# srendle/libfm

Measured on NVIDIA H100. Metric: MovieLens-1M-shaped examples/sec at k=8, SGD, higher is better.
Workload: dtype f32

## Files before the change

libfm_b200/csrc/fm_hogwild.cu:

```cuda
#include <algorithm>

#include "fm_hogwild_common.cuh"
#include "fm_rowgroup.cuh"

namespace fmb {

template <int G, int S, int R, int RW, int U, bool DAMP>
__global__ void __launch_bounds__(HW_MAX_THREADS, row_class_ctas(R, U))
    fm_sgd_hogwild_kernel(const HogwildArgs a) {
  using RG = RowGroup<G, S, R, RW>;
  constexpr int E = RG::E;
  constexpr int RPW = 32 / E;
  extern __shared__ __align__(128) unsigned char smem[];
  uint64_t* bars = reinterpret_cast<uint64_t*>(smem);
  float* s_acc = reinterpret_cast<float*>(smem + 64);

  const int tid = threadIdx.x;
  const int lane = tid & 31;
  const int warp = tid >> 5;
  const int nwarp = blockDim.x >> 5;
  const int rows_per_set = nwarp * RPW;
  const int lig = lane % E;
  const int c = lig % G;
  const int s = lig / G;
  const int sub = lane / E;
  const int TR = a.tile_rows;

  const uint64_t policy = ring_init(smem, tid);
  uint32_t* s_tile = reinterpret_cast<uint32_t*>(smem + 208);
  TileSched sched{a.sched, a.n_tiles, false};
  const int ptid = (int)blockDim.x - 32;
  uint32_t claim_raw = HW_NO_TILE;
  if (tid == ptid) {
    for (int i = 0; i < HW_NSTAGE; i++) {
      const uint32_t t = sched.claim();
      s_tile[i] = t;
      if (t != HW_NO_TILE) {
        const uint64_t r0 = (uint64_t)t * TR, r1 = min(r0 + (uint64_t)TR, a.n_rows);
        issue_tile(a, smem, bars, t, i, policy, __ldg(a.row_ptr + r0), __ldg(a.row_ptr + r1));
      }
    }
    claim_raw = sched.fire();
  }
  __syncthreads();

  const float4* V4 = reinterpret_cast<const float4*>(a.v);
  const bool use_w = a.use_w != 0;
  const bool use_w0 = a.use_w0 != 0;
  const float lr = a.lr;
  const float nlr_regv = -lr * a.regv;
  const float nlr_regw = -lr * a.regw;

  int it = 0;
  for (;; ++it) {
    const int stage = it % HW_NSTAGE;
    const uint32_t parity = (uint32_t)(it / HW_NSTAGE) & 1u;
    const uint64_t tile = s_tile[stage];
    if (tile == HW_NO_TILE) break;
    uint32_t nt = HW_NO_TILE;
    uint64_t nt_nb = 0, nt_ne = 0;
    if (tid == ptid) {
      nt = sched.resolve(claim_raw);
      claim_raw = sched.fire();
      if (nt != HW_NO_TILE) {
        const uint64_t r0 = (uint64_t)nt * TR, r1 = min(r0 + (uint64_t)TR, a.n_rows);
        nt_nb = __ldg(a.row_ptr + r0);
        nt_ne = __ldg(a.row_ptr + r1);
      }
    }
    BiasFetch bias;
    bias.slot = reinterpret_cast<float*>(smem + 192);
    bias.issue(a, use_w0, tid);
    mbar_wait(bars + stage, parity);

    unsigned char* sb = stage_base(smem, a, stage);
    const uint64_t* rp = reinterpret_cast<const uint64_t*>(sb);
    const float* ys = reinterpret_cast<const float*>(sb + (size_t)(TR + 2) * 8);
    const uint32_t* ids = reinterpret_cast<const uint32_t*>(sb + (size_t)(TR + 2) * 8 + (size_t)TR * 4);
    const float* xs = reinterpret_cast<const float*>(ids + a.tile_cap);
    const uint64_t row0 = tile * (uint64_t)TR;
    const int rows_here = (int)min((uint64_t)TR, a.n_rows - row0);
    const uint64_t ab = rp[0] & ~3ull;
    if (a.global_entries) {
      ids = a.col + ab;
      xs = a.val + ab;
    }

    float msum = 0.f, hsum = 0.f;
    float w0 = 0.f;
    bool have_w0 = false;
    for (int rbase = warp * RPW; rbase < rows_here; rbase += U * rows_per_set) {
      RG g[U];
      float y[U];
      bool valid[U];
#pragma unroll
      for (int u = 0; u < U; ++u) {
        const int r = rbase + u * rows_per_set + sub;
        valid[u] = r < rows_here;
        int beg = 0, end = 0;
        y[u] = 0.f;
        if (valid[u]) {
          beg = (int)(rp[r] - ab);
          end = (int)(rp[r + 1] - ab);
          y[u] = ys[r];
        }
        g[u].gather(V4, a.w, a.gp, a.ws, use_w, ids, xs, beg, end, c, s, lig);
      }
      if (!have_w0) {
        w0 = bias.get(use_w0, tid, it, (int)blockDim.x);
        have_w0 = true;
      }
#pragma unroll
      for (int u = 0; u < U; ++u) {
        if (U > 1 && rbase + u * rows_per_set >= rows_here) break;
        RG& gu = g[u];
        const float part = gu.template reduce<DAMP>(V4, a.w, a.gp, a.ws, use_w, ids, xs, c, s, lig);
        const LossStep ls = loss_step(a, w0 + part, y[u]);
        const float mult = ls.mult, curv = ls.curv;
        const float hjoint = DAMP ? curv * ((use_w0 ? 1.f : 0.f) + gu.hrow) : curv;
        if (valid[u] && lig == 0) {
          msum += mult;
          hsum += hjoint;
        }

        const float nlr_mult = -lr * mult;
        auto update_v = [&](int j, const float4& v) {
          const uint32_t id = ids[j];
          const float x = xs[j];
          const float x2 = x * x;
          float sv = 1.f;
          if (DAMP) {
            const float conc = __ldg(a.feat_cnt + id) * a.conc_scale;
            if (conc > 1.f) sv = gamma_scale(conc, lr * (hjoint + a.regv));
          }
          red_add_f4(a.v + ((size_t)id * a.gp + c) * 4,
                     sv * (nlr_mult * (gu.acc.x * x - v.x * x2) + nlr_regv * v.x),
                     sv * (nlr_mult * (gu.acc.y * x - v.y * x2) + nlr_regv * v.y),
                     sv * (nlr_mult * (gu.acc.z * x - v.z * x2) + nlr_regv * v.z),
                     sv * (nlr_mult * (gu.acc.w * x - v.w * x2) + nlr_regv * v.w));
        };
        if (c < a.gp) {
#pragma unroll
          for (int q = 0; q < R; ++q) {
            const int j = gu.beg + s + q * S;
            if (j < gu.end) update_v(j, gu.vc[q]);
          }
          for (int q = R; q < gu.maxit; ++q) {
            const int j = gu.beg + s + q * S;
            if (j < gu.end) update_v(j, ld_cg_f4(V4 + (size_t)ids[j] * a.gp + c));
          }
        }
        auto update_w = [&](int j, float wv) {
          const uint32_t id = ids[j];
          const float x = xs[j];
          float sw = 1.f;
          if (DAMP) {
            const float conc = __ldg(a.feat_cnt + id) * a.conc_scale;
            if (conc > 1.f) sw = gamma_scale(conc, lr * (hjoint + a.regw));
          }
          red_add_f(a.w + (size_t)id * a.ws, sw * (nlr_mult * x + nlr_regw * wv));
        };
        if (use_w) {
#pragma unroll
          for (int t = 0; t < RW; ++t) {
            const int j = gu.beg + lig + t * E;
            if (j < gu.end) update_w(j, gu.wc[t]);
          }
          for (int t = RW; t < gu.maxwit; ++t) {
            const int j = gu.beg + lig + t * E;
            if (j < gu.end) update_w(j, ld_cg_f(a.w + (size_t)ids[j] * a.ws));
          }
        }
      }
    }

    if (!have_w0) w0 = bias.get(use_w0, tid, it, (int)blockDim.x);
    float2* s_part = reinterpret_cast<float2*>(s_acc) + (it & 1) * 8;
    if (use_w0) bias_partial(s_part, msum, hsum, tid);
    __syncthreads();
    if (tid == ptid) {
      s_tile[stage] = nt;
      if (nt != HW_NO_TILE) issue_tile(a, smem, bars, nt, stage, policy, nt_nb, nt_ne);
      if (use_w0) {
        float M = 0.f, H = 0.f;
        for (int i = 0; i < nwarp; i++) {
          M += s_part[i].x;
          H += s_part[i].y;
        }
        const float T = (float)rows_here;
        M += T * a.reg0 * w0;
        const float gsc = gamma_scale(fmaxf(a.w0_conc, 1.f), lr * (H / T + a.reg0));
        red_add_f(a.w0, -lr * gsc * M);
      }
    }
  }
  if (tid == ptid) sched.finish(gridDim.x, claim_raw);
}

using KernelFn = HogwildKernelFn;

template <int G, int S, int CLS>
KernelFn pick_damp(bool damp) {
  constexpr RowClass k = row_class(CLS, G);
  return damp ? fm_sgd_hogwild_kernel<G, S, k.R, k.RW, k.U, true>
              : fm_sgd_hogwild_kernel<G, S, k.R, k.RW, k.U, false>;
}

template <int G, int S>
KernelFn pick_r(int cls, bool damp) {
  switch (cls) {
    case -1: return pick_damp<G, S, -1>(damp);
    case 0: return pick_damp<G, S, 0>(damp);
    case 1: return pick_damp<G, S, 1>(damp);
    case 2: return pick_damp<G, S, 2>(damp);
    default: return pick_damp<G, S, 3>(damp);
  }
}

void pick_geometry(int kp, uint64_t n_rows, uint64_t nnz, int* G, int* S, int* cls) {
  int gp = kp / 4;
  int g = 1;
  while (g < gp) g <<= 1;
  if (g > 32) g = 32;
  double avg = n_rows ? (double)nnz / (double)n_rows : 1.0;
  int s = 1;
  while (s < avg && s < 8) s <<= 1;
  while (g * s > 32) s >>= 1;
  if (s < 1) s = 1;
  *G = g;
  *S = s;
  const int iters = (int)((avg + s - 1) / s);
  *cls = iters <= 1 ? -1 : (iters <= 2 ? 0 : (iters <= 8 ? 1 : ((iters <= 20 || g < 32) ? 2 : 3)));
}

static bool want_damp(const fmb200_ctx* c, const DataSlot& d, double flight_per_sm) {
  const double flight_guess = std::min<double>((double)d.n_rows, (double)c->sm_count * flight_per_sm);
  const double q_max = (double)d.max_feat_cnt * flight_guess / (double)d.n_rows * c->hp.lr *
                       (1.0 + std::max(c->hp.regw, c->hp.regv));
  return c->tune_damp == 1 || (c->tune_damp == 0 && q_max > 0.5);
}

static cudaError_t fit_grid(fmb200_ctx* c, HogwildKernelFn fn, int threads, int smem, uint64_t n_tiles,
                            int* grid) {
  cudaError_t e = cudaFuncSetAttribute(fn, cudaFuncAttributeMaxDynamicSharedMemorySize, smem);
  if (e != cudaSuccess) return e;
  int occ = 0;
  e = cudaOccupancyMaxActiveBlocksPerMultiprocessor(&occ, fn, threads, smem);
  if (e != cudaSuccess) return e;
  if (occ < 1) return cudaErrorInvalidConfiguration;
  const int per_sm = c->tune_ctas_per_sm > 0 ? std::min(c->tune_ctas_per_sm, occ) : occ;
  *grid = (int)std::min<uint64_t>(n_tiles, (uint64_t)c->sm_count * per_sm);
  return cudaSuccess;
}

static HogwildArgs make_args(fmb200_ctx* c, const DataSlot& d, uint64_t n_tiles, int TR,
                             uint32_t tile_cap, uint32_t sbytes) {
  HogwildArgs a;
  a.row_ptr = d.row_ptr.get();
  a.col = d.col.get();
  a.val = d.val.get();
  a.target = d.target.get();
  a.n_rows = d.n_rows;
  a.n_tiles = (uint32_t)n_tiles;
  a.tile_rows = TR;
  a.tile_cap = tile_cap;
  a.stage_bytes = sbytes;
  a.w0 = c->p32.w0();
  a.w = c->p32.w();
  a.v = c->p32.v();
  a.gp = c->kp / 4;
  a.ws = c->p32.ws;
  a.use_w0 = c->k0;
  a.use_w = c->k1;
  a.task = c->hp.task;
  a.lr = (float)c->hp.lr;
  a.reg0 = (float)c->hp.reg0;
  a.regw = (float)c->hp.regw;
  a.regv = (float)c->hp.regv;
  a.min_target = (float)c->hp.min_target;
  a.max_target = (float)c->hp.max_target;
  a.feat_cnt = d.feat_cnt.get();
  a.conc_scale = 1.f;
  a.w0_conc = 1.f;
  a.acc_w0 = a.acc_w = a.acc_v = a.acc_bad = a.acc = nullptr;
  a.state = nullptr;
  a.n_acc = 0;
  a.ramp_tiles = 0;
  a.ramp_conc_scale = a.ramp_w0_conc = 1.f;
  a.gbar = nullptr;
  a.gbar_base = 0;
  a.prof = nullptr;
  a.deal_pos = nullptr;
  a.bias_rows = nullptr;
  a.acc_w0x = nullptr;
  a.sched = c->d_sched.get();
  a.global_entries = 0;
  return a;
}

static unsigned long long* acc_flag(fmb200_ctx* c) { return c->d_acc.get() + c->p32.n_floats; }

cudaError_t clear_acc_flag(fmb200_ctx* c) {
  return c->d_acc ? cudaMemsetAsync(acc_flag(c), 0, sizeof(unsigned long long), c->stream) : cudaSuccess;
}

struct RowlaneShape {
  HogwildKernelFn fn = nullptr;
  uint32_t cap = 0, sbytes = 0;
  int smem = 0;
};
static RowlaneShape rowlane_shape(HogwildKernelFn fn, int TR, uint32_t cap, int hdr_bytes) {
  const uint32_t sbytes = (uint32_t)hw_stage_bytes(TR, cap);
  return RowlaneShape{fn, cap, sbytes, hdr_bytes + HW_NSTAGE * (int)sbytes};
}

struct RowlanePlan {
  int threads = 0, TR = 0, launch_threads = 0, grid = 0;
  bool damp = false, combine = false, ws = false, prof = false, dealable = false;
  RowlaneShape file, dealt;
};

static cudaError_t plan_rowlane(fmb200_ctx* c, const DataSlot& d, RowlanePlan* p, bool* ok) {
  *ok = false;
  const int gp = c->kp / 4;
  if (gp < 1 || gp > 2 || d.max_row_nnz > 4 || c->tune_variant == 1 || d.n_rows == 0) return cudaSuccess;
  int threads = c->tune_threads > 0 ? std::min(c->tune_threads, HW_MAX_THREADS) : 256;
  int tr_idx = 0;
  while ((32 << (tr_idx + 1)) <= threads) tr_idx++;
  p->threads = 32 << tr_idx;
  p->TR = p->threads;
  p->damp = want_damp(c, d, 3.0 * p->TR);
  p->combine = (double)d.max_feat_cnt * 32.0 / (double)d.n_rows > 0.5;
  p->ws = c->tune_variant == 3;
  p->prof = c->tune_variant == 132 || c->tune_variant == 133;
  const uint32_t cap = (d.tile_span[tr_idx] + 3u) & ~3u;
  p->file = rowlane_shape(pick_rowlane_kernel(gp, (int)d.max_row_nnz, p->ws, p->damp, p->combine, p->prof, false),
                          p->TR, cap, p->ws ? HW_WS_HDR_BYTES : HW_HDR_BYTES);
  if (p->file.fn == nullptr) return cudaSuccess;
  p->launch_threads = p->ws ? p->threads + 32 : p->threads;
  const uint64_t n_tiles = (d.n_rows + p->TR - 1) / p->TR;
  cudaError_t e = fit_grid(c, p->file.fn, p->launch_threads, p->file.smem, n_tiles, &p->grid);
  if (e != cudaSuccess) return e;
  *ok = true;
  if (p->ws || p->combine || c->tune_variant == 5 || c->tune_variant == 133) return cudaSuccess;
  p->dealt = rowlane_shape(pick_rowlane_kernel(gp, (int)d.max_row_nnz, false, p->damp, false, p->prof, true), p->TR,
                           std::max<uint32_t>(cap, (uint32_t)p->TR * d.max_row_nnz + 4u), HW_HDR_BYTES);
  int grid_dealt = 0;
  if ((e = fit_grid(c, p->dealt.fn, p->threads, p->dealt.smem, n_tiles, &grid_dealt)) != cudaSuccess) return e;
  p->dealable = grid_dealt == p->grid;
  return cudaSuccess;
}

cudaError_t prepare_rowlane_deal(fmb200_ctx* c, DataSlot& d) {
  if (c->mode != FMB200_MODE_HOGWILD || c->kp == 0) return cudaSuccess;
  RowlanePlan p;
  bool ok = false;
  cudaError_t e = plan_rowlane(c, d, &p, &ok);
  if (e != cudaSuccess || !ok || !p.dealable) return e;
  return build_rowlane_deal(c, d, p.TR, (uint32_t)p.grid);
}

static cudaError_t launch_rowlane(fmb200_ctx* c, DataSlot& d, bool* handled) {
  *handled = false;
  RowlanePlan p;
  bool ok = false;
  cudaError_t e = plan_rowlane(c, d, &p, &ok);
  if (e != cudaSuccess || !ok) return e;
  const int TR = p.TR;
  const int grid = p.grid;
  const uint64_t n_tiles = (d.n_rows + TR - 1) / TR;
  const bool ws = p.ws;
  constexpr uint64_t kRampTiles = 4;
  const bool ramp = c->hogwild_fresh && c->k0 && c->tune_damp >= 0 && n_tiles > 8 * kRampTiles;
  c->hogwild_fresh = false;
  const bool dealt = p.dealable && !ramp && (d.deal.matches(d.upload_gen, TR, (uint32_t)grid) || d.hogwild_epochs > 0);
  d.hogwild_epochs++;
  const RowlaneShape& shape = dealt ? p.dealt : p.file;
  const HogwildKernelFn fn = shape.fn;
  const int smem = shape.smem;
  const int launch_threads = p.launch_threads;
  HogwildArgs a = make_args(c, d, n_tiles, TR, shape.cap, shape.sbytes);
  a.conc_scale = (float)(std::min<double>((double)d.n_rows, (double)grid * TR) / (double)d.n_rows);
  a.w0_conc = (float)std::min<double>((double)d.n_rows, (double)grid * TR * (ws ? HW_NSTAGE : 1));
  if (ws) {
    if (ramp) {
      HogwildArgs r = a;
      r.n_rows = kRampTiles * (uint64_t)TR;
      r.n_tiles = (uint32_t)kRampTiles;
      r.conc_scale = (float)((double)TR / (double)d.n_rows);
      r.w0_conc = (float)TR;
      fn<<<1, launch_threads, smem, c->stream>>>(r);
      c->launches++;
      const uint64_t skip = kRampTiles * (uint64_t)TR;
      a.row_ptr += skip;
      a.target += skip;
      a.n_rows -= skip;
      a.n_tiles = (uint32_t)(n_tiles - kRampTiles);
    }
    fn<<<grid, launch_threads, smem, c->stream>>>(a);
    c->launches++;
  } else {
    const uint64_t n_acc = c->p32.n_floats;
    if (n_acc % 4 != 0) return cudaErrorInvalidValue;
    if (!c->d_acc) {
      if ((e = alloc(c->d_acc, n_acc + 1)) != cudaSuccess) return e;
      e = cudaMemsetAsync(c->d_acc.get(), 0, (n_acc + 1) * sizeof(unsigned long long), c->stream);
      if (e != cudaSuccess) return e;
    }
    unsigned long long* acc = c->d_acc.get();
    float* base = c->p32.base;
    a.acc_w0 = acc + (a.w0 - base);
    a.acc_w = acc + (a.w - base);
    a.acc_v = acc + (a.v - base);
    a.acc_bad = acc_flag(c);
    a.state = base;
    a.acc = acc;
    a.n_acc = n_acc;
    if (ramp) {
      a.ramp_tiles = (uint32_t)kRampTiles;
      a.ramp_conc_scale = (float)((double)TR / (double)d.n_rows);
      a.ramp_w0_conc = (float)TR;
    }
    if (dealt) {
      if ((e = build_rowlane_deal(c, d, TR, (uint32_t)grid)) != cudaSuccess) return e;
      a.row_ptr = d.deal.row_ptr.get();
      a.col = d.deal.col.get();
      a.val = d.deal.val.get();
      a.target = d.deal.target.get();
      a.deal_pos = d.deal.pos.get();
      const uint64_t words = 2 + (uint64_t)grid * TR;
      if (c->deal_bias_cap < words) {
        if ((e = grow(c->d_deal_bias, c->deal_bias_cap, words)) != cudaSuccess) return e;
        if ((e = cudaMemsetAsync(c->d_deal_bias.get(), 0, 2 * sizeof(unsigned long long), c->stream)) != cudaSuccess)
          return e;
      }
      a.acc_w0x = c->d_deal_bias.get();
      a.bias_rows = reinterpret_cast<float2*>(c->d_deal_bias.get() + 2);
    }
    a.gbar = c->d_gbar.get();
    a.gbar_base = c->gbar_count;
    PhaseTimers prof;
    if (p.prof && (e = prof.start(RL_PROF_SLOTS, c->stream)) != cudaSuccess) return e;
    a.prof = prof.slots.get();
    void* args[] = {&a};
    e = cudaLaunchCooperativeKernel((const void*)fn, dim3(grid), dim3(launch_threads), args, (size_t)smem,
                                    c->stream);
    if (e != cudaSuccess) return e;
    c->launches++;
    const uint32_t n_win = rowlane_windows(a.n_tiles, a.ramp_tiles, (uint32_t)grid);
    c->gbar_count += (uint32_t)grid * rowlane_barriers(a.n_tiles, a.ramp_tiles, (uint32_t)grid, dealt);
    if (p.prof) {
      static const char* name[RL_PROF_SLOTS] = {"bias+gather", "score+issue", "bulk_wait", "barrier1", "fold",
                                                "barrier2"};
      if ((e = prof.print(c->stream, name, (double)n_win * grid, 1, false,
                          "[rowlane phases, cycles per window of CTA thread 0 (%u windows x %d CTAs)]", n_win,
                          grid)) != cudaSuccess)
        return e;
    }
  }
  c->last_cfg = EpochConfig{1, (int)std::max<uint32_t>(1, d.max_row_nnz), TR, grid, launch_threads, smem,
                            p.damp ? 1 : 0, dealt ? 1 : 0};
  *handled = true;
  return cudaGetLastError();
}

cudaError_t launch_sgd_hogwild(fmb200_ctx* c, DataSlot& d) {
  if (c->kp / 4 > 32) return cudaErrorInvalidValue;
  if (d.n_rows == 0) return cudaSuccess;
  {
    bool handled = false;
    cudaError_t e = launch_rowlane(c, d, &handled);
    if (e != cudaSuccess || handled) return e;
  }
  int G, S, cls;
  pick_geometry(c->kp, d.n_rows, d.nnz, &G, &S, &cls);
  const RowClass rc = row_class(cls, G);
  const int threads = c->tune_threads > 0 ? std::min(c->tune_threads, HW_MAX_THREADS) : 256;
  const int ctas_target = row_class_ctas(rc.R, rc.U);

  const int budget = (c->max_smem_optin - 1024) / ctas_target;
  int tr_idx = 3;
  if (c->tune_rows_per_tile > 0) {
    tr_idx = 0;
    while (tr_idx < 4 && (32 << (tr_idx + 1)) <= c->tune_rows_per_tile) tr_idx++;
  }
  auto stage_bytes_for = [&](int idx) {
    return hw_stage_bytes(32 << idx, ((uint64_t)d.tile_span[idx] + 3u) & ~3ull);
  };
  while (tr_idx > 0 && (uint64_t)HW_HDR_BYTES + HW_NSTAGE * stage_bytes_for(tr_idx) > (uint64_t)budget) tr_idx--;
  const bool global_entries =
      (uint64_t)HW_HDR_BYTES + (uint64_t)HW_NSTAGE * stage_bytes_for(tr_idx) > (uint64_t)c->max_smem_optin;
  if (global_entries) tr_idx = 1;
  const int TR = 32 << tr_idx;
  const uint32_t cap = global_entries ? 0u : (d.tile_span[tr_idx] + 3u) & ~3u;
  const uint32_t sbytes = (uint32_t)hw_stage_bytes(TR, cap);
  const int smem = HW_HDR_BYTES + HW_NSTAGE * (int)sbytes;

  const double rows_per_cta_step = (double)(threads / 32) * (32.0 / (G * S)) * rc.U;
  const bool damp = want_damp(c, d, ctas_target * rows_per_cta_step);

  const KernelFn fn = dispatch_gs(G, S, [&](auto g, auto s) { return pick_r<g, s>(cls, damp); });
  const uint64_t n_tiles = (d.n_rows + TR - 1) / TR;
  int grid = 0;
  cudaError_t e = fit_grid(c, fn, threads, smem, n_tiles, &grid);
  if (e != cudaSuccess) return e;

  HogwildArgs a = make_args(c, d, n_tiles, TR, cap, sbytes);
  a.global_entries = global_entries ? 1 : 0;
  a.conc_scale = (float)(std::min<double>((double)d.n_rows, (double)grid * rows_per_cta_step) /
                         (double)d.n_rows);
  a.w0_conc = (float)std::min<double>((double)d.n_rows, (double)grid * TR);
  fn<<<grid, threads, smem, c->stream>>>(a);
  c->launches++;
  c->last_cfg = EpochConfig{G, S, TR, grid, threads, smem, damp ? 1 : 0};
  return cudaGetLastError();
}

}
```

libfm_b200/csrc/fm_hogwild_common.cuh:

```cuda
#pragma once
#include "fm_device.cuh"
#include "fmb200_internal.h"

namespace fmb {

constexpr int HW_NSTAGE = 3;
constexpr int HW_MAX_THREADS = 256;
constexpr uint32_t HW_NO_TILE = 0xffffffffu;
constexpr int HW_HDR_BYTES = 256;
constexpr int HW_WS_HDR_BYTES = 512;

template <typename T>
__host__ __device__ inline T hw_rp_bytes(int TR) { return (T)(TR + 2) * 8; }
template <typename T>
__host__ __device__ inline T hw_y_bytes(int TR) { return (T)TR * 4; }
__host__ __device__ inline uint64_t hw_stage_bytes(int TR, uint64_t cap) {
  return (hw_rp_bytes<uint64_t>(TR) + hw_y_bytes<uint64_t>(TR) + 2 * cap * 4 + 15) & ~15ull;
}

struct HogwildArgs {
  const uint64_t* row_ptr;
  const uint32_t* col;
  const float* val;
  const float* target;
  uint64_t n_rows;
  uint32_t n_tiles;
  int tile_rows;
  uint32_t tile_cap;
  uint32_t stage_bytes;
  float* w0;
  float* w;
  float* v;
  int gp;
  int ws;
  int use_w0, use_w, task;
  float lr, reg0, regw, regv, min_target, max_target;
  const float* feat_cnt;
  float conc_scale;
  float w0_conc;
  unsigned int* sched;
  int global_entries;
  unsigned long long *acc_w0, *acc_w, *acc_v;
  unsigned long long* acc_bad;
  float* state;
  unsigned long long* acc;
  uint64_t n_acc;
  uint32_t ramp_tiles;
  float ramp_conc_scale, ramp_w0_conc;
  unsigned int* gbar;
  uint32_t gbar_base;
  unsigned long long* prof;
  const uint32_t* deal_pos;
  float2* bias_rows;
  unsigned long long* acc_w0x;
};

__host__ __device__ inline uint32_t rowlane_windows(uint32_t n_tiles, uint32_t ramp, uint32_t G) {
  return ramp + (n_tiles - ramp + G - 1) / G;
}
__host__ __device__ inline uint32_t rowlane_barriers(uint32_t n_tiles, uint32_t ramp, uint32_t G, bool dealt) {
  return 2u * rowlane_windows(n_tiles, ramp, G) - (dealt ? 0u : 1u);
}

struct GridBarrier {
  unsigned int* count;
  uint32_t target;
  __device__ __forceinline__ void arrive(int tid) {
    __syncthreads();
    if (tid == 0) red_release_add_u32(count, 1u);
    target += gridDim.x;
  }
  __device__ __forceinline__ void wait(int tid) {
    if (tid == 0)
      while ((int32_t)(ld_acquire_u32(count) - target) < 0) {
      }
    __syncthreads();
  }
};

constexpr float kAccScale = 0x1p32f;
constexpr float kAccStepMax = 0x1p11f;

__device__ __forceinline__ void acc_add(unsigned long long* p, float d, unsigned long long* bad) {
  if (fabsf(d) < kAccStepMax) red_add_u64(p, (unsigned long long)__float2ll_rn(d * kAccScale));
  else atomicOr(bad, 1ull);
}
__device__ __forceinline__ unsigned long long acc_quantise(float d, unsigned long long* bad) {
  if (fabsf(d) < kAccStepMax) return (unsigned long long)__float2ll_rn(d * kAccScale);
  atomicOr(bad, 1ull);
  return 0ull;
}

__device__ __forceinline__ float acc_fold(float x, unsigned long long u, bool bad) {
  if (bad) return __int_as_float(0x7fffffff);
  return u != 0ull ? x + (float)((double)(long long)u * (1.0 / (double)kAccScale)) : x;
}

__device__ __forceinline__ unsigned char* stage_base(unsigned char* smem, const HogwildArgs& a,
                                                     int stage, int hdr = HW_HDR_BYTES) {
  return smem + hdr + (size_t)stage * a.stage_bytes;
}

__device__ __forceinline__ void issue_tile(const HogwildArgs& a, unsigned char* smem, uint64_t* bars,
                                           uint32_t tile, int stage, uint64_t policy, uint64_t nb,
                                           uint64_t ne, int hdr = HW_HDR_BYTES) {
  const int TR = a.tile_rows;
  const uint64_t r0 = (uint64_t)tile * TR;
  const uint64_t ab = nb & ~3ull;
  const uint64_t ae = (ne + 3ull) & ~3ull;
  const uint32_t ebytes = a.global_entries ? 0u : (uint32_t)(ae - ab) * 4u;
  const uint32_t rp_bytes = hw_rp_bytes<uint32_t>(TR);
  const uint32_t y_bytes = hw_y_bytes<uint32_t>(TR);
  unsigned char* sb = stage_base(smem, a, stage, hdr);
  uint64_t* bar = bars + stage;
  mbar_arrive_expect_tx(bar, rp_bytes + y_bytes + 2u * ebytes);
  bulk_g2s_hint(sb, a.row_ptr + r0, rp_bytes, bar, policy);
  bulk_g2s_hint(sb + rp_bytes, a.target + r0, y_bytes, bar, policy);
  if (ebytes) {
    unsigned char* cb = sb + rp_bytes + y_bytes;
    bulk_g2s_hint(cb, a.col + ab, ebytes, bar, policy);
    bulk_g2s_hint(cb + (size_t)a.tile_cap * 4u, a.val + ab, ebytes, bar, policy);
  }
}

__device__ __forceinline__ uint64_t ring_init(unsigned char* smem, int tid) {
  uint64_t* bars = reinterpret_cast<uint64_t*>(smem);
  uint64_t policy = 0;
  if (tid == 0) {
    for (int i = 0; i < HW_NSTAGE; i++) mbar_init(bars + i, 1);
    fence_mbar_init();
  }
  if (tid == (int)blockDim.x - 32) policy = policy_evict_first();
  __syncthreads();
  return policy;
}

struct LossStep {
  float mult, curv;
};
__device__ __forceinline__ LossStep loss_step(const HogwildArgs& a, float p, float y) {
  LossStep l;
  if (a.task == FMB200_TASK_REGRESSION) {
    const float pc = fmaxf(a.min_target, fminf(a.max_target, p));
    l.mult = pc - y;
    const float den = p - y;
    l.curv = (pc == p) ? 1.f : (fabsf(den) > 1e-12f ? fminf(fmaxf(l.mult / den, 0.f), 1.f) : 0.f);
  } else {
    const float sg = 1.f / (1.f + __expf(-y * p));
    l.mult = -y * (1.f - sg);
    l.curv = sg * (1.f - sg);
  }
  return l;
}

__device__ __forceinline__ float gamma_scale(float c, float u) {
  if (c <= 1.f || u <= 0.f) return 1.f;
  const float q = c * u;
  if (q < 1e-3f) return 1.f;
  const float a = fmaxf(1.f - u, 0.f);
  const float ac = a > 0.f ? __expf(c * __logf(a)) : 0.f;
  return fminf(1.f, (1.f - ac) / q);
}

__device__ __forceinline__ void bias_partial(float2* part, float mult, float hjoint, int tid) {
  mult = warp_sum(mult);
  hjoint = warp_sum(hjoint);
  if ((tid & 31) == 0) part[tid >> 5] = make_float2(mult, hjoint);
}

struct BiasFetch {
  float* slot;
  float pending;
  __device__ __forceinline__ void issue(const HogwildArgs& a, bool use_w0, int tid) {
    pending = 0.f;
    if (use_w0 && tid == 0) pending = ld_cg_f(a.w0);
  }
  __device__ __forceinline__ float get(bool use_w0, int tid, int it, int nthreads) {
    if (!use_w0) return 0.f;
    float* s = slot + (it & 1);
    if (tid < 32) {
      const float v = __shfl_sync(0xffffffffu, pending, 0);
      if (tid == 0) *s = v;
      __threadfence_block();
      named_bar_arrive(1, nthreads);
      return v;
    }
    named_bar_sync(1, nthreads);
    return *s;
  }
};

struct TileSched {
  unsigned int* w;
  uint32_t n_tiles;
  bool dry;
  __device__ __forceinline__ uint32_t claim() {
    if (dry) return HW_NO_TILE;
    const uint32_t t = atomicAdd(w, 1u);
    if (t >= n_tiles) {
      dry = true;
      return HW_NO_TILE;
    }
    return t;
  }
  __device__ __forceinline__ uint32_t fire() { return dry ? HW_NO_TILE : atomicAdd(w, 1u); }
  __device__ __forceinline__ uint32_t resolve(uint32_t raw) {
    if (raw >= n_tiles) {
      dry = true;
      return HW_NO_TILE;
    }
    return raw;
  }
  __device__ __forceinline__ void finish(unsigned int n_ctas, uint32_t last_raw) {
    unsigned int inc = (last_raw == 0x7fffffffu) ? 2u : 1u;
    __threadfence();
    if (atomicAdd(w + 1, inc) == n_ctas - 1) {
      w[0] = 0u;
      w[1] = 0u;
    }
  }
};

using HogwildKernelFn = void (*)(const HogwildArgs);

HogwildKernelFn pick_rowlane_kernel(int gp, int max_row_nnz, bool ws, bool damp, bool combine, bool prof, bool dealt);
constexpr int RL_PROF_SLOTS = 6;

}
```

libfm_b200/csrc/fm_rowlane.cu:

```cuda
#include <algorithm>

#include "fm_hogwild_common.cuh"

namespace fmb {

template <int GP>
struct FactorRow {
  float v[4 * GP];
};

template <int GP>
__device__ __forceinline__ unsigned long long* wb_slot(int e, int tid) {
  __shared__ __align__(128) unsigned long long s_wb[2][HW_MAX_THREADS][4 * GP];
  return s_wb[e & 1][tid];
}
template <int GP, int Z, typename Q>
__device__ __forceinline__ void acc_add_row_q(unsigned long long* acc_v, uint32_t id, bool live, int e, int tid, Q q) {
  constexpr int K = 4 * GP;
  unsigned long long* slot = wb_slot<GP>(e, tid);
  bulk_wait_read<Z == 1 ? 0 : 1>();
  if (live) {
#pragma unroll
    for (int f = 0; f < K; f += 2) *reinterpret_cast<ulonglong2*>(slot + f) = make_ulonglong2(q(f), q(f + 1));
    fence_proxy_async_shared();
    bulk_red_add_u64(acc_v + (size_t)id * K, slot, K * 8);
  }
  bulk_commit();
}
template <int GP, int Z>
__device__ __forceinline__ void acc_add_row(unsigned long long* acc_v, uint32_t id, bool live,
                                            const float (&d)[4 * GP], int e, int tid, unsigned long long* bad) {
  acc_add_row_q<GP, Z>(acc_v, id, live, e, tid, [&](int f) { return acc_quantise(d[f], bad); });
}

template <int GP>
__device__ __forceinline__ FactorRow<GP> gather_row(const float4* V4, uint32_t gid, int odd) {
  FactorRow<GP> r;
  const float4 zero4 = make_float4(0.f, 0.f, 0.f, 0.f);
  if constexpr (GP == 2) {
    const uint32_t pid = __shfl_xor_sync(0xffffffffu, gid, 1);
    const uint32_t idA = odd ? pid : gid;
    const uint32_t idB = odd ? gid : pid;
    const float4 la = idA != 0xffffffffu ? ld_cg_f4(V4 + (size_t)idA * 2 + odd) : zero4;
    const float4 lb = idB != 0xffffffffu ? ld_cg_f4(V4 + (size_t)idB * 2 + odd) : zero4;
    const float4 send = odd ? la : lb;
    float4 recv;
    recv.x = __shfl_xor_sync(0xffffffffu, send.x, 1);
    recv.y = __shfl_xor_sync(0xffffffffu, send.y, 1);
    recv.z = __shfl_xor_sync(0xffffffffu, send.z, 1);
    recv.w = __shfl_xor_sync(0xffffffffu, send.w, 1);
    const float4 lo = odd ? recv : la;
    const float4 hi = odd ? lb : recv;
    r.v[0] = lo.x; r.v[1] = lo.y; r.v[2] = lo.z; r.v[3] = lo.w;
    r.v[4] = hi.x; r.v[5] = hi.y; r.v[6] = hi.z; r.v[7] = hi.w;
  } else {
    const float4 l = gid != 0xffffffffu ? ld_cg_f4(V4 + (size_t)gid) : zero4;
    r.v[0] = l.x; r.v[1] = l.y; r.v[2] = l.z; r.v[3] = l.w;
  }
  return r;
}

template <int GP, int Z, bool DAMP, bool COMBINE, bool ACC, bool DEALT, typename W0F>
__device__ __forceinline__ void rowlane_tile(const HogwildArgs& a, const uint64_t* rp,
                                             const float* ys, const uint32_t* ids,
                                             const float* xs, int rows_here, int tid, W0F get_w0,
                                             float& mult_out, float& hjoint_out) {
  constexpr int K = 4 * GP;
  const int lane = tid & 31;
  const int odd = lane & 1;
  const float4* V4 = reinterpret_cast<const float4*>(a.v);
  const bool use_w = a.use_w != 0;
  const bool use_w0 = a.use_w0 != 0;
  const float lr = a.lr;
  const uint64_t ab = rp[0] & ~3ull;
  const bool valid = tid < rows_here;
  int beg = 0, cnt = 0;
  float y = 0.f;
  if (valid) {
    beg = (int)(rp[tid] - ab);
    cnt = (int)(rp[tid + 1] - ab) - beg;
    y = ys[tid];
  }
  uint32_t id[Z];
  float x[Z], wv[Z];
  FactorRow<GP> vr[Z];
#pragma unroll
  for (int e = 0; e < Z; ++e) {
    const bool on = e < cnt;
    id[e] = on ? ids[beg + e] : 0u;
    x[e] = on ? xs[beg + e] : 0.f;
  }
  const int kq = DEALT ? cnt - 1 : -1;
  uint32_t kid = 0xffffffffu;
#pragma unroll
  for (int e = 0; e < Z; ++e)
    if (e == kq) kid = id[e];
  int seg = lane;
  if (DEALT) {
    const uint32_t prev = __shfl_up_sync(0xffffffffu, kid, 1);
    const bool head = lane == 0 || kid == 0xffffffffu || prev != kid;
    seg = 31 - __clz(__ballot_sync(0xffffffffu, head) & (0xffffffffu >> (31 - lane)));
  }
#pragma unroll
  for (int e = 0; e < Z; ++e) {
    const bool fetch = e < cnt && e != kq;
    vr[e] = gather_row<GP>(V4, fetch ? id[e] : 0xffffffffu, odd);
    wv[e] = (use_w && fetch) ? ld_cg_f(a.w + (size_t)id[e] * a.ws) : 0.f;
  }
  if (DEALT) {
    const bool fetch = lane == seg && kid != 0xffffffffu;
    FactorRow<GP> kv = gather_row<GP>(V4, fetch ? kid : 0xffffffffu, odd);
    float kw = (use_w && fetch) ? ld_cg_f(a.w + (size_t)kid * a.ws) : 0.f;
#pragma unroll
    for (int f = 0; f < K; ++f) kv.v[f] = __shfl_sync(0xffffffffu, kv.v[f], seg);
    kw = __shfl_sync(0xffffffffu, kw, seg);
#pragma unroll
    for (int e = 0; e < Z; ++e)
      if (e == kq) {
        vr[e] = kv;
        wv[e] = kw;
      }
  }

  float sum[K];
#pragma unroll
  for (int f = 0; f < K; ++f) sum[f] = 0.f;
  float sq = 0.f, lin = 0.f, xx = 0.f;
#pragma unroll
  for (int e = 0; e < Z; ++e) {
#pragma unroll
    for (int f = 0; f < K; ++f) {
      const float d = vr[e].v[f] * x[e];
      sum[f] += d;
      sq += d * d;
    }
    lin += wv[e] * x[e];
    xx += x[e] * x[e];
  }
  float s2 = 0.f;
#pragma unroll
  for (int f = 0; f < K; ++f) s2 += sum[f] * sum[f];
  const float w0 = get_w0();
  const float p = w0 + lin + 0.5f * (s2 - sq);

  const LossStep ls = loss_step(a, p, y);
  float mult = ls.mult, curv = ls.curv;
  if (!valid) {
    mult = 0.f;
    curv = 0.f;
  }
  const float hrow = (use_w ? xx : 0.f) + fmaxf((xx - 2.f) * s2 + sq, 0.f);
  const float hjoint = DAMP ? curv * ((use_w0 ? 1.f : 0.f) + hrow) : curv;

  struct KeyStep {
    float v[K], w;
  } kd{};
  auto make_kd = [](const float (&d)[K], float dw) {
    KeyStep k;
#pragma unroll
    for (int f = 0; f < K; ++f) k.v[f] = d[f];
    k.w = dw;
    return k;
  };
  const float nlr_mult = -lr * mult;
  const float nlr_regv = -lr * a.regv;
  const float nlr_regw = -lr * a.regw;
#pragma unroll
  for (int e = 0; e < Z; ++e) {
    const bool on = e < cnt;
    float sv = 1.f, sw = 1.f;
    if (DAMP) {
      const float conc = on ? __ldg(a.feat_cnt + id[e]) * a.conc_scale : 0.f;
      if (conc > 1.f) {
        sv = gamma_scale(conc, lr * (hjoint + a.regv));
        sw = gamma_scale(conc, lr * (hjoint + a.regw));
      }
    }
    const float x2 = x[e] * x[e];
    float d[K];
#pragma unroll
    for (int f = 0; f < K; ++f)
      d[f] = sv * (nlr_mult * (sum[f] * x[e] - vr[e].v[f] * x2) + nlr_regv * vr[e].v[f]);
    float dw = sw * (nlr_mult * x[e] + nlr_regw * wv[e]);
    bool on_c = on;
    if (DEALT && e == kq) {
      kd = make_kd(d, dw);
      on_c = false;
    }
    if (COMBINE) {
      const uint32_t key = on ? id[e] : (0x80000000u | (uint32_t)lane);
      unsigned peers = __match_any_sync(0xffffffffu, key);
      if (__any_sync(0xffffffffu, __popc(peers) > 1)) {
        const int first = __ffs(peers) - 1;
        int rel = __popc(peers << (31 - lane) << 1);
        peers &= (0xfffffffeu << lane);
        while (__any_sync(0xffffffffu, peers != 0u)) {
          const int next = __ffs(peers);
          const int src = next ? next - 1 : lane;
#pragma unroll
          for (int f = 0; f < K; ++f) {
            const float t = __shfl_sync(0xffffffffu, d[f], src);
            if (next) d[f] += t;
          }
          const float tw = __shfl_sync(0xffffffffu, dw, src);
          if (next) dw += tw;
          const unsigned done = __ballot_sync(0xffffffffu, rel & 1);
          peers &= ~done;
          rel >>= 1;
        }
        on_c = on && (lane == first);
      }
    }
    if constexpr (ACC) {
      acc_add_row<GP, Z>(a.acc_v, id[e], on_c, d, e, tid, a.acc_bad);
    } else if (GP == 2) {
      const uint32_t pid = __shfl_xor_sync(0xffffffffu, id[e], 1);
      const bool pon = __shfl_xor_sync(0xffffffffu, (int)on_c, 1) != 0;
      const uint32_t idA = odd ? pid : id[e];
      const uint32_t idB = odd ? id[e] : pid;
      const bool onA = odd ? pon : on_c;
      const bool onB = odd ? on_c : pon;
      float4 send, keep;
      if (odd) {
        send = make_float4(d[0], d[1], d[2], d[3]);
        keep = make_float4(d[4], d[5], d[6], d[7]);
      } else {
        send = make_float4(d[4], d[5], d[6], d[7]);
        keep = make_float4(d[0], d[1], d[2], d[3]);
      }
      float4 recv;
      recv.x = __shfl_xor_sync(0xffffffffu, send.x, 1);
      recv.y = __shfl_xor_sync(0xffffffffu, send.y, 1);
      recv.z = __shfl_xor_sync(0xffffffffu, send.z, 1);
      recv.w = __shfl_xor_sync(0xffffffffu, send.w, 1);
      const float4 va = odd ? recv : keep;
      const float4 vb = odd ? keep : recv;
      if (onA) red_add_f4(a.v + ((size_t)idA * 2 + odd) * 4, va.x, va.y, va.z, va.w);
      if (onB) red_add_f4(a.v + ((size_t)idB * 2 + odd) * 4, vb.x, vb.y, vb.z, vb.w);
    } else if (on_c) {
      red_add_f4(a.v + (size_t)id[e] * 4, d[0], d[1], d[2], d[3]);
    }
    if (on_c && use_w) {
      if (ACC) acc_add(a.acc_w + (size_t)id[e] * a.ws, dw, a.acc_bad);
      else red_add_f(a.w + (size_t)id[e] * a.ws, dw);
    }
  }
  if constexpr (DEALT) {
    const bool has_key = kid != 0xffffffffu;
    unsigned long long q[K + 1];
#pragma unroll
    for (int f = 0; f < K; ++f) q[f] = has_key ? acc_quantise(kd.v[f], a.acc_bad) : 0ull;
    q[K] = (has_key && use_w) ? acc_quantise(kd.w, a.acc_bad) : 0ull;
#pragma unroll
    for (int s = 1; s < 32; s <<= 1) {
      const bool take = __shfl_down_sync(0xffffffffu, seg, s) == seg && lane + s < 32;
#pragma unroll
      for (int f = 0; f <= K; ++f) {
        const unsigned long long t = __shfl_down_sync(0xffffffffu, q[f], s);
        if (take) q[f] += t;
      }
    }
    const bool issue = has_key && lane == seg;
    acc_add_row_q<GP, Z>(a.acc_v, kid, issue, Z, tid, [&](int f) { return q[f]; });
    if (issue && use_w) red_add_u64(a.acc_w + (size_t)kid * a.ws, q[K]);
  }

  mult_out = mult;
  hjoint_out = valid ? hjoint : 0.f;
}

constexpr int RL_PROF_OFF = 200;

template <int GP, int Z, bool DAMP, bool COMBINE, bool PROF, bool DEALT>
__global__ void __launch_bounds__(HW_MAX_THREADS, 3) fm_sgd_rowlane_kernel(const HogwildArgs a) {
  extern __shared__ __align__(128) unsigned char smem[];
  uint64_t* bars = reinterpret_cast<uint64_t*>(smem);
  float* s_acc = reinterpret_cast<float*>(smem + 64);
  unsigned long long* s_prof = reinterpret_cast<unsigned long long*>(smem + RL_PROF_OFF);

  const int tid = threadIdx.x;
  const int TR = a.tile_rows;
  const uint32_t G = gridDim.x;
  const uint32_t R = a.ramp_tiles;
  const uint32_t n_win = rowlane_windows(a.n_tiles, R, G);
  long long tprof = 0;
  auto prof_mark = [&](int slot) {
    if constexpr (PROF) {
      if (tid == 0) {
        const long long now = clock64();
        s_prof[slot] += (unsigned long long)(now - tprof);
        tprof = now;
      }
    }
  };
  if (PROF && tid < RL_PROF_SLOTS) s_prof[tid] = 0ull;
  auto tile_of = [&](uint32_t j) -> uint32_t {
    const uint32_t t = j < R ? (blockIdx.x == 0 ? j : HW_NO_TILE) : R + (j - R) * G + blockIdx.x;
    return t < a.n_tiles ? t : HW_NO_TILE;
  };

  const uint64_t policy = ring_init(smem, tid);
  const int ptid = (int)blockDim.x - 32;
  uint32_t pj = 0;
  auto next_tile = [&]() -> uint32_t {
    for (; pj < n_win; ++pj)
      if (tile_of(pj) != HW_NO_TILE) return tile_of(pj++);
    return HW_NO_TILE;
  };
  if (tid == ptid) {
    for (int i = 0; i < HW_NSTAGE; i++) {
      const uint32_t t = next_tile();
      if (t != HW_NO_TILE) {
        const uint64_t r0 = (uint64_t)t * TR, r1 = min(r0 + (uint64_t)TR, a.n_rows);
        issue_tile(a, smem, bars, t, i, policy, __ldg(a.row_ptr + r0), __ldg(a.row_ptr + r1));
      }
    }
  }
  __syncthreads();

  const bool use_w0 = a.use_w0 != 0;
  const float lr = a.lr;
  GridBarrier gbar{a.gbar, a.gbar_base};
  const uint64_t q0 = blockIdx.x * (uint64_t)blockDim.x + tid;
  const uint64_t fold_stride = (uint64_t)G * blockDim.x;
  const uint64_t n_vec = a.n_acc / 4;
  float4* state4 = reinterpret_cast<float4*>(a.state);
  ulonglong2* acc2 = reinterpret_cast<ulonglong2*>(a.acc);
  if (PROF && tid == 0) tprof = clock64();

  float w0_run = (DEALT && use_w0 && tid == 0) ? ld_cg_f(a.w0) : 0.f;
  bool bad = false;
  int it = 0;
  for (uint32_t j = 0; j < n_win; ++j) {
    const uint32_t tile = tile_of(j);
    if (DEALT && use_w0 && tid == 0 && j > 0) w0_run = acc_fold(w0_run, __ldcg(a.acc_w0x + ((j - 1) & 1)), bad);
    if (tile != HW_NO_TILE) {
      const int stage = it % HW_NSTAGE;
      const uint32_t parity = (uint32_t)(it / HW_NSTAGE) & 1u;
      uint32_t nt = HW_NO_TILE;
      uint64_t nt_nb = 0, nt_ne = 0;
      if (tid == ptid) {
        nt = next_tile();
        if (nt != HW_NO_TILE) {
          const uint64_t r0 = (uint64_t)nt * TR, r1 = min(r0 + (uint64_t)TR, a.n_rows);
          nt_nb = __ldg(a.row_ptr + r0);
          nt_ne = __ldg(a.row_ptr + r1);
        }
      }
      HogwildArgs w = a;
      if (j < R) {
        w.conc_scale = a.ramp_conc_scale;
        w.w0_conc = a.ramp_w0_conc;
      }
      BiasFetch bias;
      bias.slot = reinterpret_cast<float*>(smem + 192);
      if (DEALT) bias.pending = w0_run;
      else bias.issue(a, use_w0, tid);
      const uint32_t pos = DEALT && tid < (int)min((uint64_t)TR, a.n_rows - (uint64_t)tile * TR)
                               ? __ldg(a.deal_pos + (uint64_t)tile * TR + tid)
                               : 0xffffffffu;
      mbar_wait(bars + stage, parity);

      unsigned char* sb = stage_base(smem, a, stage);
      const uint64_t* rp = reinterpret_cast<const uint64_t*>(sb);
      const float* ys = reinterpret_cast<const float*>(sb + (size_t)(TR + 2) * 8);
      const uint32_t* ids = reinterpret_cast<const uint32_t*>(sb + (size_t)(TR + 2) * 8 + (size_t)TR * 4);
      const float* xs = reinterpret_cast<const float*>(ids + a.tile_cap);
      const uint64_t row0 = (uint64_t)tile * TR;
      const int rows_here = (int)min((uint64_t)TR, a.n_rows - row0);

      float mult, hj, w0 = 0.f;
      rowlane_tile<GP, Z, DAMP, COMBINE, true, DEALT>(
          w, rp, ys, ids, xs, rows_here, tid,
          [&]() {
            w0 = bias.get(use_w0, tid, it, (int)blockDim.x);
            prof_mark(0);
            return w0;
          },
          mult, hj);
      float2* s_part = reinterpret_cast<float2*>(s_acc) + (it & 1) * 8;
      if (DEALT) {
        if (use_w0 && pos != 0xffffffffu) a.bias_rows[pos] = make_float2(mult, hj);
      } else if (use_w0) {
        bias_partial(s_part, mult, hj, tid);
      }
      __syncthreads();
      if (tid == ptid) {
        if (nt != HW_NO_TILE) issue_tile(a, smem, bars, nt, stage, policy, nt_nb, nt_ne);
        if (!DEALT && use_w0) {
          float M = 0.f, H = 0.f;
          for (int i = 0; i < (int)(blockDim.x >> 5); i++) {
            M += s_part[i].x;
            H += s_part[i].y;
          }
          const float T = (float)rows_here;
          M += T * a.reg0 * w0;
          const float gsc = gamma_scale(fmaxf(w.w0_conc, 1.f), lr * (H / T + a.reg0));
          acc_add(a.acc_w0, -lr * gsc * M, a.acc_bad);
        }
      }
      ++it;
    }
    prof_mark(1);
    bulk_wait_all();
    fence_proxy_async_global();
    gbar.arrive(tid);
    prof_mark(2);
    float4 s = make_float4(0.f, 0.f, 0.f, 0.f);
    if (q0 < n_vec) s = __ldcg(state4 + q0);
    gbar.wait(tid);
    prof_mark(3);
    float2 pr = make_float2(0.f, 0.f);
    if (DEALT && use_w0 && tile != HW_NO_TILE && tid < (int)min((uint64_t)TR, a.n_rows - (uint64_t)tile * TR))
      pr = __ldcg(a.bias_rows + blockIdx.x * TR + tid);
    bad = __ldcg(a.acc + a.n_acc) != 0ull;
    for (uint64_t q = q0; q < n_vec; q += fold_stride) {
      const ulonglong2 lo = __ldcg(acc2 + 2 * q), hi = __ldcg(acc2 + 2 * q + 1);
      if (q != q0) s = __ldcg(state4 + q);
      s.x = acc_fold(s.x, lo.x, bad);
      s.y = acc_fold(s.y, lo.y, bad);
      s.z = acc_fold(s.z, hi.x, bad);
      s.w = acc_fold(s.w, hi.y, bad);
      if (bad || (lo.x | lo.y | hi.x | hi.y) != 0ull) state4[q] = s;
      if ((lo.x | lo.y) != 0ull) acc2[2 * q] = make_ulonglong2(0ull, 0ull);
      if ((hi.x | hi.y) != 0ull) acc2[2 * q + 1] = make_ulonglong2(0ull, 0ull);
    }
    if (DEALT && use_w0) {
      if (tile != HW_NO_TILE) {
        float2* s_part = reinterpret_cast<float2*>(s_acc);
        bias_partial(s_part, pr.x, pr.y, tid);
        __syncthreads();
        if (tid == 0) {
          float M = 0.f, H = 0.f;
          for (int i = 0; i < (int)(blockDim.x >> 5); i++) {
            M += s_part[i].x;
            H += s_part[i].y;
          }
          const float T = (float)min((uint64_t)TR, a.n_rows - (uint64_t)tile * TR);
          M += T * a.reg0 * w0_run;
          const float gsc = gamma_scale(fmaxf(a.w0_conc, 1.f), lr * (H / T + a.reg0));
          acc_add(a.acc_w0x + (j & 1), -lr * gsc * M, a.acc_bad);
        }
      }
      if (blockIdx.x == 0 && tid == 0 && j > 0) a.acc_w0x[(j - 1) & 1] = 0ull;
    }
    prof_mark(4);
    if (DEALT || j + 1 < n_win) {
      gbar.arrive(tid);
      gbar.wait(tid);
    }
    fence_proxy_async_global();
    prof_mark(5);
  }
  if (DEALT) {
    const bool bad_end = __ldcg(a.acc + a.n_acc) != 0ull;
    if (bad_end && !bad)
      for (uint64_t q = q0; q < n_vec; q += fold_stride) state4[q] = make_float4(NAN, NAN, NAN, NAN);
    if (use_w0 && blockIdx.x == 0 && tid == 0) {
      *a.w0 = acc_fold(w0_run, __ldcg(a.acc_w0x + ((n_win - 1) & 1)), bad_end);
      a.acc_w0x[(n_win - 1) & 1] = 0ull;
    }
  }
  if constexpr (PROF) {
    __syncthreads();
    if (tid < RL_PROF_SLOTS) atomicAdd(a.prof + tid, s_prof[tid]);
  }
}


__device__ __forceinline__ void mbar_arrive(uint64_t* bar) {
  asm volatile("mbarrier.arrive.shared::cta.b64 _, [%0];" ::"r"(smem_u32(bar)) : "memory");
}

template <int GP, int Z, bool DAMP, bool COMBINE>
__global__ void __launch_bounds__(HW_MAX_THREADS + 32, 3) fm_sgd_rowlane_ws_kernel(const HogwildArgs a) {
  extern __shared__ __align__(128) unsigned char smem[];
  uint64_t* full = reinterpret_cast<uint64_t*>(smem);
  uint64_t* empty = reinterpret_cast<uint64_t*>(smem + 64);
  uint32_t* s_tile = reinterpret_cast<uint32_t*>(smem + 128);
  float* s_w0 = reinterpret_cast<float*>(smem + 160);
  float2* s_part = reinterpret_cast<float2*>(smem + 192);

  const int tid = threadIdx.x;
  const int lane = tid & 31;
  const int TR = a.tile_rows;
  const int n_cwarps = TR >> 5;
  const bool use_w0 = a.use_w0 != 0;
  auto stage_ptr = [&](int stage) { return smem + HW_WS_HDR_BYTES + (size_t)stage * a.stage_bytes; };

  if (tid == 0) {
    for (int i = 0; i < HW_NSTAGE; i++) {
      mbar_init(full + i, 1);
      mbar_init(empty + i, (uint32_t)n_cwarps);
    }
    fence_mbar_init();
  }
  __syncthreads();

  if (tid >= TR) {
    if (lane != 0) return;
    TileSched sched{a.sched, a.n_tiles, false};
    const uint64_t policy = policy_evict_first();
    auto fill = [&](int stage, uint32_t t) {
      s_tile[stage] = t;
      if (t == HW_NO_TILE) {
        mbar_arrive(full + stage);
        return;
      }
      s_w0[stage] = use_w0 ? ld_cg_f(a.w0) : 0.f;
      const uint64_t r0 = (uint64_t)t * TR, r1 = min(r0 + (uint64_t)TR, a.n_rows);
      issue_tile(a, smem, full, t, stage, policy, __ldg(a.row_ptr + r0), __ldg(a.row_ptr + r1), HW_WS_HDR_BYTES);
    };
    for (int i = 0; i < HW_NSTAGE; i++) fill(i, sched.claim());
    for (int it = 0;; ++it) {
      const int stage = it % HW_NSTAGE;
      const uint32_t t = s_tile[stage];
      if (t == HW_NO_TILE) break;
      mbar_wait(empty + stage, (uint32_t)(it / HW_NSTAGE) & 1u);
      if (use_w0) {
        float M = 0.f, H = 0.f;
        for (int i = 0; i < n_cwarps; i++) {
          const float2 p = s_part[stage * 8 + i];
          M += p.x;
          H += p.y;
        }
        const uint64_t row0 = (uint64_t)t * TR;
        const float T = (float)min((uint64_t)TR, a.n_rows - row0);
        M += T * a.reg0 * s_w0[stage];
        const float gsc = gamma_scale(fmaxf(a.w0_conc, 1.f), a.lr * (H / T + a.reg0));
        red_add_f(a.w0, -a.lr * gsc * M);
      }
      fill(stage, sched.claim());
    }
    sched.finish(gridDim.x, 0u);
    return;
  }

  for (int it = 0;; ++it) {
    const int stage = it % HW_NSTAGE;
    mbar_wait(full + stage, (uint32_t)(it / HW_NSTAGE) & 1u);
    const uint32_t tile = s_tile[stage];
    if (tile == HW_NO_TILE) break;
    unsigned char* sb = stage_ptr(stage);
    const uint64_t* rp = reinterpret_cast<const uint64_t*>(sb);
    const float* ys = reinterpret_cast<const float*>(sb + (size_t)(TR + 2) * 8);
    const uint32_t* ids = reinterpret_cast<const uint32_t*>(sb + (size_t)(TR + 2) * 8 + (size_t)TR * 4);
    const float* xs = reinterpret_cast<const float*>(ids + a.tile_cap);
    const uint64_t row0 = (uint64_t)tile * TR;
    const int rows_here = (int)min((uint64_t)TR, a.n_rows - row0);
    const float w0 = s_w0[stage];
    float mult, hj;
    rowlane_tile<GP, Z, DAMP, COMBINE, false, false>(a, rp, ys, ids, xs, rows_here, tid, [&]() { return w0; }, mult,
                                                     hj);
    if (use_w0) bias_partial(s_part + stage * 8, mult, hj, tid);
    __syncwarp();
    if (lane == 0) mbar_arrive(empty + stage);
  }
}

template <auto... Vs, class T, class F>
static HogwildKernelFn dispatch(T v, F f) {
  HogwildKernelFn fn = nullptr;
  (void)((v == Vs && (fn = f(std::integral_constant<decltype(Vs), Vs>{}), true)) || ...);
  return fn;
}

HogwildKernelFn pick_rowlane_kernel(int gp, int max_row_nnz, bool ws, bool damp, bool combine, bool prof, bool dealt) {
  const int z = max_row_nnz <= 1 ? 1 : (max_row_nnz <= 2 ? 2 : (max_row_nnz <= 4 ? 4 : 0));
  return dispatch<1, 2>(gp, [&](auto GP) {
    return dispatch<1, 2, 4>(z, [&](auto Z) {
      return dispatch<false, true>(damp, [&](auto D) {
        return dispatch<false, true>(combine, [&](auto C) {
          if (ws) return fm_sgd_rowlane_ws_kernel<GP, Z, D, C>;
          return dispatch<false, true>(prof, [&](auto P) {
            return dispatch<false, true>(dealt, [&](auto DL) -> HogwildKernelFn {
              if constexpr (DL && C) return nullptr;
              else return fm_sgd_rowlane_kernel<GP, Z, D, C, P, DL>;
            });
          });
        });
      });
    });
  });
}

}
```

Before: 6.883 billion.

## Move dealt-mode w0 bias reduction off the grid barrier critical path

In the dealt rowlane path, each CTA's global-bias partial reduction now runs between the grid barrier's arrive and wait, so it overlaps barrier latency. A per-window arrival counter is added, and each CTA spins on it before folding the previous window's w0 accumulator. The fold is deferred into the bias fetch callback instead of happening at window start. This takes the per-window w0 reduction out of the serialized barrier phase, at the cost of an extra counter, spin-waits, and added complexity in resetting the counters.

```diff
diff --git a/libfm_b200/csrc/fm_hogwild.cu b/libfm_b200/csrc/fm_hogwild.cu
--- a/libfm_b200/csrc/fm_hogwild.cu
+++ b/libfm_b200/csrc/fm_hogwild.cu
@@ -293,6 +293,7 @@
   a.deal_pos = nullptr;
   a.bias_rows = nullptr;
   a.acc_w0x = nullptr;
+  a.w0x_count = nullptr;
   a.sched = c->d_sched.get();
   a.global_entries = 0;
   return a;
@@ -428,14 +429,15 @@
       a.val = d.deal.val.get();
       a.target = d.deal.target.get();
       a.deal_pos = d.deal.pos.get();
-      const uint64_t words = 2 + (uint64_t)grid * TR;
+      const uint64_t words = 3 + (uint64_t)grid * TR;
       if (c->deal_bias_cap < words) {
         if ((e = grow(c->d_deal_bias, c->deal_bias_cap, words)) != cudaSuccess) return e;
-        if ((e = cudaMemsetAsync(c->d_deal_bias.get(), 0, 2 * sizeof(unsigned long long), c->stream)) != cudaSuccess)
+        if ((e = cudaMemsetAsync(c->d_deal_bias.get(), 0, 3 * sizeof(unsigned long long), c->stream)) != cudaSuccess)
           return e;
       }
       a.acc_w0x = c->d_deal_bias.get();
-      a.bias_rows = reinterpret_cast<float2*>(c->d_deal_bias.get() + 2);
+      a.w0x_count = reinterpret_cast<unsigned int*>(c->d_deal_bias.get() + 2);
+      a.bias_rows = reinterpret_cast<float2*>(c->d_deal_bias.get() + 3);
     }
     a.gbar = c->d_gbar.get();
     a.gbar_base = c->gbar_count;
diff --git a/libfm_b200/csrc/fm_hogwild_common.cuh b/libfm_b200/csrc/fm_hogwild_common.cuh
--- a/libfm_b200/csrc/fm_hogwild_common.cuh
+++ b/libfm_b200/csrc/fm_hogwild_common.cuh
@@ -53,6 +53,7 @@
   const uint32_t* deal_pos;
   float2* bias_rows;
   unsigned long long* acc_w0x;
+  unsigned int* w0x_count;
 };
 
 __host__ __device__ inline uint32_t rowlane_windows(uint32_t n_tiles, uint32_t ramp, uint32_t G) {
diff --git a/libfm_b200/csrc/fm_rowlane.cu b/libfm_b200/csrc/fm_rowlane.cu
--- a/libfm_b200/csrc/fm_rowlane.cu
+++ b/libfm_b200/csrc/fm_rowlane.cu
@@ -333,7 +333,14 @@
   int it = 0;
   for (uint32_t j = 0; j < n_win; ++j) {
     const uint32_t tile = tile_of(j);
-    if (DEALT && use_w0 && tid == 0 && j > 0) w0_run = acc_fold(w0_run, __ldcg(a.acc_w0x + ((j - 1) & 1)), bad);
+    auto advance_w0 = [&]() {
+      if (DEALT && use_w0 && tid == 0 && j > 0) {
+        while (ld_acquire_u32(a.w0x_count + ((j - 1) & 1)) < G) {
+        }
+        w0_run = acc_fold(w0_run, __ldcg(a.acc_w0x + ((j - 1) & 1)), bad);
+      }
+    };
+    if (tile == HW_NO_TILE) advance_w0();
     if (tile != HW_NO_TILE) {
       const int stage = it % HW_NSTAGE;
       const uint32_t parity = (uint32_t)(it / HW_NSTAGE) & 1u;
@@ -354,8 +361,7 @@
       }
       BiasFetch bias;
       bias.slot = reinterpret_cast<float*>(smem + 192);
-      if (DEALT) bias.pending = w0_run;
-      else bias.issue(a, use_w0, tid);
+      if (!DEALT) bias.issue(a, use_w0, tid);
       const uint32_t pos = DEALT && tid < (int)min((uint64_t)TR, a.n_rows - (uint64_t)tile * TR)
                                ? __ldg(a.deal_pos + (uint64_t)tile * TR + tid)
                                : 0xffffffffu;
@@ -373,6 +379,10 @@
       rowlane_tile<GP, Z, DAMP, COMBINE, true, DEALT>(
           w, rp, ys, ids, xs, rows_here, tid,
           [&]() {
+            if (DEALT) {
+              advance_w0();
+              bias.pending = w0_run;
+            }
             w0 = bias.get(use_w0, tid, it, (int)blockDim.x);
             prof_mark(0);
             return w0;
@@ -425,7 +435,7 @@
       if ((lo.x | lo.y) != 0ull) acc2[2 * q] = make_ulonglong2(0ull, 0ull);
       if ((hi.x | hi.y) != 0ull) acc2[2 * q + 1] = make_ulonglong2(0ull, 0ull);
     }
-    if (DEALT && use_w0) {
+    auto bias_step = [&]() {
       if (tile != HW_NO_TILE) {
         float2* s_part = reinterpret_cast<float2*>(s_acc);
         bias_partial(s_part, pr.x, pr.y, tid);
@@ -442,11 +452,20 @@
           acc_add(a.acc_w0x + (j & 1), -lr * gsc * M, a.acc_bad);
         }
       }
-      if (blockIdx.x == 0 && tid == 0 && j > 0) a.acc_w0x[(j - 1) & 1] = 0ull;
+      if (tid == 0) red_release_add_u32(a.w0x_count + (j & 1), 1u);
+    };
+    const bool late_step = DEALT && use_w0 && j + 1 < n_win;
+    if (DEALT && use_w0) {
+      if (blockIdx.x == 0 && tid == 0 && j > 0) {
+        a.acc_w0x[(j - 1) & 1] = 0ull;
+        a.w0x_count[(j - 1) & 1] = 0u;
+      }
+      if (!late_step) bias_step();
     }
     prof_mark(4);
     if (DEALT || j + 1 < n_win) {
       gbar.arrive(tid);
+      if (late_step) bias_step();
       gbar.wait(tid);
     }
     fence_proxy_async_global();
@@ -459,6 +478,7 @@
     if (use_w0 && blockIdx.x == 0 && tid == 0) {
       *a.w0 = acc_fold(w0_run, __ldcg(a.acc_w0x + ((n_win - 1) & 1)), bad_end);
       a.acc_w0x[(n_win - 1) & 1] = 0ull;
+      a.w0x_count[(n_win - 1) & 1] = 0u;
     }
   }
   if constexpr (PROF) {
```

New measurement: 7.006 billion, median of 6. 1.02x the previous value.
